# hidasib/GRU4Rec

Hardware: NVIDIA H100
Metric: mini-batches/sec (higher is better)
Workload: dtype f32

## Files before the change

### gru4rec_b200/csrc/g4r_fast.cuh

```cuda
#pragma once

constexpr int FK_THREADS = 512;
constexpr int FK_NW = FK_THREADS / 32;
constexpr int FK_G = 48;
constexpr int FK_CT = 32;
constexpr int FK_Q = FK_CT / FK_NW;
constexpr int FK_B = 32;
static_assert(FK_THREADS / 16 == FK_B, "statistics mapping: 16 threads per lane");
constexpr int FK_LDS = 132;


__device__ __forceinline__ void red_release_add(unsigned int* p, unsigned int v) {
  asm volatile("red.release.gpu.global.add.u32 [%0], %1;" :: "l"(p), "r"(v) : "memory");
}
__device__ __forceinline__ unsigned int atom_acqrel_add(unsigned int* p, unsigned int v) {
  unsigned int old;
  asm volatile("atom.acq_rel.gpu.global.add.u32 %0, [%1], %2;" : "=r"(old) : "l"(p), "r"(v) : "memory");
  return old;
}
__device__ __forceinline__ void wait_ge(const unsigned int* p, unsigned int target) {
  while (ld_acquire_u32(p) < target) { }
}
__device__ __forceinline__ uint32_t smem_u32(const void* p) { return (uint32_t)__cvta_generic_to_shared(p); }
__device__ __forceinline__ void mbar_init(uint64_t* bar, unsigned int count) {
// ... 604 lines not shown
  }
}
template <class SM>
__device__ __forceinline__ void fk_dsy(SM& sm, int M, int nj, int kw) {
  for (int t = threadIdx.x; t < nj * kw; t += FK_THREADS) {
    const int jj = t / kw, q4 = t % kw;
    float4 d = make_float4(0.f, 0.f, 0.f, 0.f);
    for (int bb = 0; bb < M; bb++) {
      const float4 y = ld4(sm.sY + bb * FK_LDS + q4 * 4);
      const float g = sm.sG[jj * FK_B + bb];
      d.x = fmaf(g, y.x, d.x); d.y = fmaf(g, y.y, d.y); d.z = fmaf(g, y.z, d.z); d.w = fmaf(g, y.w, d.w);
    }
    st4(sm.sD + jj * FK_LDS + q4 * 4, d);
  }
}
template <class SM>
__device__ __forceinline__ void fk_update_rows(const ModelDev& md, SM& sm, int buf, int nj, int kw) {
  const int lane = threadIdx.x & 31, warp = threadIdx.x >> 5, ldL = md.ldL;
  const bool ada = md.adapt == G4R_ADAPT_ADAGRAD, mom = md.mom > 0.f;
  for (int j = warp; j < nj; j += FK_NW) {
    const int item = sm.sIt[buf][j];
    if (j > 0 && sm.sIt[buf][j - 1] == item) continue;
    int je = j + 1;
    while (je < nj && sm.sIt[buf][je] == item) je++;
    if (lane < kw) {
      const float4 p0 = ld4(sm.sS + j * FK_LDS + lane * 4), z = make_float4(0.f, 0.f, 0.f, 0.f);
      RowChain<float4> u;
      u.begin(p0, p0, ada ? ld4(sm.sAcc + j * FK_LDS + lane * 4) : z, mom ? ld4(sm.sVel + j * FK_LDS + lane * 4) : z);
      for (int k = j; k < je; k++) u.add(md, ld4(sm.sD + k * FK_LDS + lane * 4), ada, mom);
      const size_t off = (size_t)item * ldL + lane * 4;
      st4(md.Wy + off, u.ps);
      if (ada) st4(md.Wy_acc + off, u.al);
      if (mom) st4(md.Wy_vel + off, u.vl);
    }
    if (lane == 0) {
      RowChain<float> u;
      u.begin(sm.sByP[j], sm.sByP[j], sm.sByA[j], sm.sByV[j]);
      for (int k = j; k < je; k++) u.add(md, sm.sDby[k], ada, mom);
      md.By[item] = u.ps;
      if (ada) md.By_acc[item] = u.al;
      if (mom) md.By_vel[item] = u.vl;
    }
  }
}
template <class SM>
__device__ __forceinline__ void fk_dby(SM& sm, int M, int nj) {
  const int lane = threadIdx.x & 31, warp = threadIdx.x >> 5;
  for (int jj = warp; jj < nj; jj += FK_NW) {
    float a = (lane < M) ? sm.sG[jj * FK_B + lane] : 0.f;
    a = warp_sum(a);
    if (lane == 0) sm.sDby[jj] = a;
  }
}
struct FkPartner { int nj, it; float g[2]; };
__device__ __forceinline__ FkPartner fk_partner_fetch(const ModelDev& md, int s, int g, int M) {
  const int tid = threadIdx.x;
  const int* cbeg = md.pCbeg + (size_t)s * (md.NCH + 1);
  const int cb = g < md.NCH ? cbeg[g] : 0;
  FkPartner r;
  r.nj = g < md.NCH ? cbeg[g + 1] - cb : 0;
  r.it = (tid < r.nj) ? md.pItem[(size_t)s * md.NP + cb + tid] : 0;
#pragma unroll
  for (int u = 0; u < 2; u++) {
    const int i = u * FK_THREADS + tid, jj = i / FK_B, b = i % FK_B;
    r.g[u] = (jj < r.nj && b < M) ? md.O[(size_t)(cb + jj) * md.Bld + b] : 0.f;
  }
  return r;
}
template <class SM>
__device__ int fk_partner_stage(const ModelDev& md, SM& sm, const FkPartner& r, int buf, int M, int kw) {
  static_assert(FK_CT * FK_B == 2 * FK_THREADS, "fk_partner_fetch: two dL/do entries per thread");
  const int tid = threadIdx.x, lane = tid & 31, warp = tid >> 5, nj = r.nj;
  const bool ada = md.adapt == G4R_ADAPT_ADAGRAD, mom = md.mom > 0.f;
  __syncthreads();
  if (tid < FK_CT) sm.sIt[buf][tid] = r.it;
  sm.sG[tid] = r.g[0]; sm.sG[FK_THREADS + tid] = r.g[1];
  __syncthreads();
  for (int j = warp; j < nj; j += FK_NW) {
    const int it = sm.sIt[buf][j];
    const size_t off = (size_t)it * md.ldL + lane * 4;
    if (lane < kw) {
      st4(sm.sS + j * FK_LDS + lane * 4, ld4(md.Wy + off));
      if (ada) st4(sm.sAcc + j * FK_LDS + lane * 4, ld4(md.Wy_acc + off));
      if (mom) st4(sm.sVel + j * FK_LDS + lane * 4, ld4(md.Wy_vel + off));
    }
    if (lane == 0) { sm.sByP[j] = md.By[it]; sm.sByA[j] = ada ? md.By_acc[it] : 0.f; sm.sByV[j] = mom ? md.By_vel[it] : 0.f; }
  }
  asm volatile("fence.proxy.async.shared::cta;" ::: "memory");
  fk_dby(sm, M, nj);
  return nj;
}

#include "g4r_fastc.cuh"

template <bool CL>
__global__ void __launch_bounds__(FK_THREADS, 1) k_fast_t(int slot, int n_steps, FastSync* fs, unsigned long long* tstamp) {
  using SM = typename std::conditional<CL, FastSmemC, FastSmemR>::type;
  extern __shared__ __align__(128) unsigned char fk_raw[];
  SM& sm = *reinterpret_cast<SM*>(fk_raw);
  const ModelDev& md = MD;
  const LayerDev& ly = md.layer[0];
  const int cta = blockIdx.x, ncta = gridDim.x;
  const int tid = threadIdx.x, lane = tid & 31, warp = tid >> 5;
  const int chunk = cta;
  const bool has_chunk = chunk < md.NCH;
  const int G = CL ? (int)cl_size() : md.ldL / 4;
  const bool gru = cta < G;
  const bool pw = loss_pairwise(md.loss);
  const int ldL = md.ldL, B = md.B;
  const int kw = ldL / 4;
  uint64_t* bar = reinterpret_cast<uint64_t*>(&sm.mbar);
  unsigned int bar_epoch = 0, gepoch = 0, stats_target = 0;
  const int in_ctas = min(B, ncta - G);
  const int partner_of = (!CL && cta >= G + in_ctas && cta < 2 * G + in_ctas) ? cta - G - in_ctas : -1;
#ifdef G4R_CF_FINE
#define FK_FTS(s_) ((tstamp && cta == 0 && (s_) < 500 && n_steps >= 1000) ? tstamp + (size_t)((s_) + 500) * 16 : nullptr)
#define FK_STAMP_OK(s_) ((s_) < 500)
#else
#define FK_FTS(s_) ((unsigned long long*)nullptr)
#define FK_STAMP_OK(s_) true
#endif
#define FK_STAMP(k) do { if (tstamp && cta == 0 && tid == 0 && FK_STAMP_OK(s)) { unsigned long long t_; asm volatile("mov.u64 %0, %%globaltimer;" : "=l"(t_)); tstamp[(size_t)s * 16 + (k)] = t_; } } while (0)
  if (tid == 0) { mbar_init(bar, 1); asm volatile("fence.mbarrier_init.release.cluster;" ::: "memory"); }
  fk_load_idx(md, sm, 0, n_steps, chunk, 0);
  __syncthreads();
  fk_prefetch_rows(md, sm, 0, n_steps, 0, pw);
  ClusterCtx cc = {0, 1, 0, 0};
  if constexpr (CL) {
    if (gru) {
      cc = cf_init(md, sm);
      cf_load_resident(md, sm, cc);
      if (n_steps > 0) {
        fk_stage_lanes(md, sm, 0, md.wM[0]);
        cf_f1(md, sm, cc, 0, false, nullptr, 0u, nullptr);
        cf_f2(md, sm, cc, 0, nullptr);
        __syncthreads();
        if (tid == 0) red_release_add(&fs->h_ready, 1u);
      }
    }
  } else {
    if (gru) {
      fr_load_resident(md, sm, 4 * cta);
      if (n_steps > 0) {
        fk_stage_lanes(md, sm, 0, md.wM[0]);
        stage_rows4(sm.gH[0], FK_LDS, FK_B, kw, [&](int rr) -> const float* { const int sl = sm.gIdx[rr]; return sl >= 0 ? ly.H + (size_t)sl * ldL : nullptr; });
        fr_f1(md, sm, 0, 4 * cta, sm.gH[0], nullptr, 0u);
        fk_group_barrier(fs, gepoch, G);
        fr_f2(md, sm, 0, 4 * cta, sm.gH[0]);
        __syncthreads();
        if (tid == 0) red_release_add(&fs->h_ready, 1u);
      }
    }
  }
  for (int s = 0; s < n_steps; s++) {
    const int buf = s & 1;
    const int M = md.wM[s];
    const int sti = md.wSti[s];
    const int N = M + (sti >= 0 ? md.S : 0);
    FK_STAMP(0);
    fk_load_idx(md, sm, s + 1, n_steps, chunk, buf ^ 1);
    const bool gru_next = !CL && gru && s + 1 < n_steps;
    if (gru_next && tid < FK_B) {
      const int M1 = md.wM[s + 1];
      sm.gIdx[tid] = tid < M1 ? md.wSlot[(size_t)(s + 1) * B + tid] : -1;
      sm.gIdx[FK_B + tid] = tid < M1 ? md.wX[(size_t)(s + 1) * B + tid] : 0;
      sm.gIdx[2 * FK_B + tid] = tid < M1 ? md.wF[(size_t)(s + 1) * B + tid] : 0;
    }
    if (tid == 0) wait_ge(&fs->h_ready, (unsigned int)(s + 1) * (unsigned int)G);
    __syncthreads();
    stage_rows4(sm.sY, FK_LDS, FK_B, kw, [&](int rr) -> const float* { return rr < M ? ly.y + (size_t)rr * ldL : nullptr; });
    mbar_wait(bar, (unsigned int)(s & 1));
    __syncthreads();
    FK_STAMP(1);
    const int cb = sm.sCb[buf][0], ce = sm.sCb[buf][1];
    const int nj = ce - cb;
    if (pw) {
      for (int b = warp; b < FK_B; b += FK_NW) {
        if (b < M) {
          float a = 0.f;
          if (lane < kw) {
            const float4 y = ld4(sm.sY + b * FK_LDS + lane * 4), w = ld4(sm.sTW + b * FK_LDS + lane * 4);
            a = fmaf(w.x, y.x, a); a = fmaf(w.y, y.y, a); a = fmaf(w.z, y.z, a); a = fmaf(w.w, y.w, a);
          }
          a = warp_sum(a);
          if (lane == 0) sm.sT[b] = act_fwd(md.fact, a + sm.sTB[b]);
        }
      }
    }
    {
      float accq[FK_Q];
#pragma unroll
      for (int q = 0; q < FK_Q; q++) accq[q] = 0.f;
      const float* yr = sm.sY + lane * FK_LDS;
      for (int c4 = 0; c4 < kw; c4++) {
        const float4 y = ld4(yr + c4 * 4);
#pragma unroll
        for (int q = 0; q < FK_Q; q++) {
          if (warp + FK_NW * q < nj) {
            const float4 w = ld4(sm.sS + (warp + FK_NW * q) * FK_LDS + c4 * 4);
            accq[q] = fmaf(y.x, w.x, accq[q]); accq[q] = fmaf(y.y, w.y, accq[q]); accq[q] = fmaf(y.z, w.z, accq[q]); accq[q] = fmaf(y.w, w.w, accq[q]);
          }
        }
      }
      FK_STAMP(9);
#pragma unroll
      for (int q = 0; q < FK_Q; q++) {
        const int jj = warp + q * FK_NW;
        if (jj < nj && lane < M) sm.sO[jj * FK_B + lane] = accq[q] + sm.sBias[jj];
      }
      __syncthreads();
      {
        const int b = tid >> 4, sub = tid & 15;
        const bool okb = b < M;
        const int tc = okb ? sm.sTc[buf][b] : -1;
        const float t = (pw && okb) ? sm.sT[b] : 0.f;
        float yv[2]; bool use[2], ist[2];
        float mloc = -INFINITY;
        const bool smx = loss_softmaxneg(md.loss), xe = (md.loss == G4R_LOSS_XE || md.loss == G4R_LOSS_XE_LOGIT);
#pragma unroll
        for (int q = 0; q < 2; q++) {
          const int jj = sub + 16 * q;
          use[q] = okb && jj < nj;
          ist[q] = use[q] && (tc == cb + jj);
          const float o = use[q] ? sm.sO[jj * FK_B + b] : 0.f;
          yv[q] = xe ? o : act_fwd(md.fact, o);
          if (use[q] && (xe || (smx && !ist[q]))) mloc = fmaxf(mloc, yv[q]);
        }
#pragma unroll
        for (int o = 1; o < 16; o <<= 1) mloc = fmaxf(mloc, __shfl_xor_sync(0xffffffffu, mloc, o));
        float Z = 0.f, A = 0.f, Q = 0.f, D = 0.f, T = 0.f, has = 0.f;
#pragma unroll
        for (int q = 0; q < 2; q++) {
          if (!use[q]) continue;
          const float y = yv[q];
          if (ist[q]) has = 1.f;
          if (xe) { Z += expf(y - mloc); if (ist[q]) T = y; }
          else if (md.loss == G4R_LOSS_BPR_MAX) { if (!ist[q]) { const float e = expf(y - mloc), sg = sigmoidf_(t - y); Z += e; A += sg * e; Q += y * y * e; D += sg * (1.f - sg) * e; } }
          else if (md.loss == G4R_LOSS_TOP1_MAX) { if (!ist[q]) { const float e = expf(y - mloc), a1 = sigmoidf_(y - t), b1 = sigmoidf_(y * y); Z += e; A += (a1 + b1) * e; D += a1 * (1.f - a1) * e; } }
          else if (md.loss == G4R_LOSS_BPR) { const float sg = sigmoidf_(t - y); A += -logf(sg); if (!ist[q]) D += 1.f - sg; }
          else { const float a1 = sigmoidf_(y - t), b1 = sigmoidf_(y * y); A += a1 + b1; if (!ist[q]) D += a1 * (1.f - a1); }
        }
#pragma unroll
        for (int o = 1; o < 16; o <<= 1) {
          Z += __shfl_xor_sync(0xffffffffu, Z, o); A += __shfl_xor_sync(0xffffffffu, A, o); Q += __shfl_xor_sync(0xffffffffu, Q, o);
          D += __shfl_xor_sync(0xffffffffu, D, o); T += __shfl_xor_sync(0xffffffffu, T, o); has += __shfl_xor_sync(0xffffffffu, has, o);
        }
        if (has_chunk && okb && sub == 0) {
          float* st = md.stat + ((size_t)chunk * md.B + b) * G4R_NSTAT;
          st4(st, make_float4(mloc, Z, A, Q));
          st4(st + 4, make_float4(D, T, has > 0.f ? 1.f : 0.f, pw ? t : 0.f));
        }
      }
    }
    __syncthreads();
    FK_STAMP(10);
    bar_epoch += 1;
    if (tid == 0) { red_release_add(&fs->bar, 1u); wait_ge(&fs->bar, bar_epoch * (unsigned int)ncta); }
    __syncthreads();
    if (cta < M) {
      const int b = cta;
      const bool maxed = !(md.loss == G4R_LOSS_BPR || md.loss == G4R_LOSS_TOP1);
      float mc = -INFINITY, Z = 0.f, A = 0.f, Q = 0.f, D = 0.f, T = 0.f, has = 0.f, tt = 0.f;
      if (tid < md.NCH) {
        const float* st = md.stat + ((size_t)tid * md.B + b) * G4R_NSTAT;
        const float4 u = ld4(st), v = ld4(st + 4);
        mc = u.x; Z = u.y; A = u.z; Q = u.w; D = v.x; T = v.y; has = v.z;
        if (tid == 0) tt = v.w;
      }
      float mg = mc;
#pragma unroll
      for (int o = 1; o < 32; o <<= 1) mg = fmaxf(mg, __shfl_xor_sync(0xffffffffu, mg, o));
      if (lane == 0) sm.sPart[warp] = mg;
      __syncthreads();
      mg = sm.sPart[0];
      for (int w = 1; w < FK_NW; w++) mg = fmaxf(mg, sm.sPart[w]);
      if (loss_softmaxneg(md.loss)) mg = fmaxf(mg, 0.f);
      if (maxed) {
        const float sc = (mc == -INFINITY) ? 0.f : expf(mc - mg);
        Z *= sc; A *= sc; Q *= sc; D *= sc;
      }
#pragma unroll
      for (int o = 1; o < 32; o <<= 1) {
        Z += __shfl_xor_sync(0xffffffffu, Z, o); A += __shfl_xor_sync(0xffffffffu, A, o); Q += __shfl_xor_sync(0xffffffffu, Q, o);
        D += __shfl_xor_sync(0xffffffffu, D, o); T += __shfl_xor_sync(0xffffffffu, T, o); has += __shfl_xor_sync(0xffffffffu, has, o);
      }
      __syncthreads();
      if (lane == 0) { float* w = sm.sPart + 32 + warp * 8; w[0] = Z; w[1] = A; w[2] = Q; w[3] = D; w[4] = T; w[5] = has; w[6] = tt; }
      __syncthreads();
      if (tid == 0) {
        tt = sm.sPart[32 + 6];
        for (int w = 1; w < FK_NW; w++) { const float* q = sm.sPart + 32 + w * 8; Z += q[0]; A += q[1]; Q += q[2]; D += q[3]; T += q[4]; }
        const float m = mg;
        float* rs = md.RS + (size_t)b * G4R_NSTAT;
        float loss = 0.f, r0 = m, r1 = Z, r2 = 0.f, r3 = 0.f, r4 = 0.f, r5 = tt;
        if (md.loss == G4R_LOSS_XE) { const float pt = __fdiv_rn(expf(T - m), Z); loss = -logf(pt + G4R_EPS_LOG); r2 = pt; r5 = T; }
        else if (md.loss == G4R_LOSS_XE_LOGIT) { loss = logf(Z) - (T - m); r5 = T; }
        else if (md.loss == G4R_LOSS_BPR_MAX) { r2 = __fdiv_rn(A, Z); r3 = __fdiv_rn(Q, Z); r4 = __fdiv_rn(D, Z); loss = -logf(r2 + G4R_EPS_LOG) + md.bpreg * r3; }
        else if (md.loss == G4R_LOSS_TOP1_MAX) { r2 = __fdiv_rn(A, Z); r4 = __fdiv_rn(D, Z); loss = r2; }
        else if (md.loss == G4R_LOSS_BPR) { loss = A; r4 = D; }
        else { const float c = sigmoidf_(tt * tt); loss = (float)M * (__fdiv_rn(A, (float)N) - __fdiv_rn(c, (float)(M + md.S_cfg))); r4 = D; }
        st4(rs, make_float4(r0, r1, r2, r3));
        st4(rs + 4, make_float4(r4, r5, loss, 0.f));
        red_release_add(&fs->stats, 1u);
      }
    }
    stats_target += (unsigned int)M;
    if (tid == 0) wait_ge(&fs->stats, stats_target);
    __syncthreads();
    FK_STAMP(2);
    if (tid < M * 2) st4(sm.sRS + tid * 4, ld4(md.RS + tid * 4));
    __syncthreads();
    if (chunk == 0 && tid == 0) {
      float c = 0.f;
      for (int b = 0; b < M; b++) c += sm.sRS[b * 8 + 6];
      c = __fdiv_rn(c, (float)md.B);
      md.cost[s] = c;
      if (c != c) atomicExch(md.nanflag, 1);
    }
    FK_STAMP(11);
    for (int i = tid; i < FK_CT * FK_B; i += FK_THREADS) {
      const int jj = i / FK_B, b = i % FK_B;
      sm.sG[i] = (jj < nj && b < M) ? loss_grad_elem(md, sm.sRS + (size_t)b * 8, sm.sO[i], sm.sTc[buf][b] == cb + jj, M, N) : 0.f;
    }
    __syncthreads();
    if (!CL && gru) {
      for (int i = tid; i < nj * FK_B; i += FK_THREADS) {
        const int jj = i / FK_B, b = i % FK_B;
        if (b < M) md.O[(size_t)(cb + jj) * md.Bld + b] = sm.sG[i];
      }
    } else {
      fk_dby(sm, M, nj);
    }
    FK_STAMP(12);
    float* part = md.part + (size_t)(has_chunk ? chunk : 0) * md.B * ldL;
    if constexpr (CL) {
      if (has_chunk) { fk_dsy(sm, M, nj, kw); fk_part(sm, part, M, nj, ldL); }
      __syncthreads();
      FK_STAMP(13);
      fk_update_rows(md, sm, buf, nj, kw);
      if (has_chunk && nj == 0) for (int i = tid; i < M * ldL; i += FK_THREADS) part[i] = 0.f;
      __syncthreads();
      FK_STAMP(14);
      bar_epoch += 1;
      if (tid == 0) { red_release_add(&fs->bar, 1u); wait_ge(&fs->bar, bar_epoch * (unsigned int)ncta); }
      __syncthreads();
      FK_STAMP(3);
      fk_b1<CL>(md, sm, s, cta, ncta);
      __syncthreads();
      if (tid == 0) red_release_add(&fs->b1_done, 1u);
      FK_STAMP(15);
      fk_prefetch_rows(md, sm, s + 1, n_steps, buf ^ 1, pw);
      FK_STAMP(4);
      if (gru) {
        if (s + 1 < n_steps) fk_stage_lanes(md, sm, s + 1, md.wM[s + 1]);
        cf_backward(md, sm, cc, fs, s, ncta, s + 1 < n_steps, (tstamp && cta == 0 && FK_STAMP_OK(s)) ? tstamp + (size_t)s * 16 : nullptr, FK_FTS(s));
        FK_STAMP(6);
        if (s + 1 < n_steps) {
          cf_f1(md, sm, cc, s + 1, true, &fs->in_done, (unsigned int)(s + 1) * (unsigned int)in_ctas, FK_FTS(s));
          FK_STAMP(7);
          cf_f2(md, sm, cc, s + 1, FK_FTS(s));
          __syncthreads();
          if (tid == 0) red_release_add(&fs->h_ready, 1u);
        } else {
          cl_wait();
        }
        FK_STAMP(8);
      }
      if (!gru && cta < G + in_ctas) {
        const unsigned int tgt = (unsigned int)(s + 1) * (unsigned int)G;
        if (in_ctas == B && ly.ld3 / 4 <= FK_THREADS) fk_sparse_in_one(md, sm, s, cta - G, &fs->grp, tgt);
        else {
          if (tid == 0) wait_ge(&fs->grp, tgt);
          __syncthreads();
          for (int b = cta - G; b < B; b += in_ctas) { fk_sparse_in(md, sm, s, b); __syncthreads(); }
        }
        __syncthreads();
        if (tid == 0) red_release_add(&fs->in_done, 1u);
      }
    } else {
      if (has_chunk) fk_part(sm, part, M, nj, ldL);
      if (has_chunk && nj == 0) for (int i = tid; i < M * ldL; i += FK_THREADS) part[i] = 0.f;
      __syncthreads();
      FK_STAMP(13);
      bar_epoch += 1;
      if (tid == 0) { red_release_add(&fs->bar, 1u); wait_ge(&fs->bar, bar_epoch * (unsigned int)ncta); }
      __syncthreads();
      FK_STAMP(3);
      fk_b1<CL>(md, sm, s, cta, ncta);
      __syncthreads();
      if (tid == 0) red_release_add(&fs->b1_done, 1u);
      FK_STAMP(15);
      const bool nxt = s + 1 < n_steps;
      const unsigned int rows_target = (unsigned int)(s + 1) * (unsigned int)ncta;
      if (gru) {
        const int k0 = 4 * cta;
        const float* sHo = sm.gH[s & 1];
        float* hnext = sm.gH[(s + 1) & 1];
        if (nxt) stage_rows4(hnext, FK_LDS, FK_B, kw, [&](int rr) -> const float* { const int sl = sm.gIdx[rr]; return sl >= 0 ? ly.H + (size_t)sl * ldL : nullptr; });
        __syncthreads();
        FK_STAMP(14);
        if (tid == 0) { red_release_add(&fs->rows_done, 1u); wait_ge(&fs->b1_done, (unsigned int)(s + 1) * (unsigned int)ncta); }
        __syncthreads();
        FK_STAMP(4);
        fr_b2(md, sm, s, k0, sHo);
        __syncthreads();
        if (tid == 0) red_release_add(&fs->dvec_done, 1u);
        FK_STAMP(5);
        fr_dense(md, sm, s, k0, sHo);
        FK_STAMP(6);
        if (nxt) {
          fr_f1(md, sm, s + 1, k0, hnext, &fs->in_done, (unsigned int)(s + 1) * (unsigned int)in_ctas);
          fk_group_barrier(fs, gepoch, G);
          FK_STAMP(7);
          fr_f2(md, sm, s + 1, k0, hnext);
          __syncthreads();
          if (tid == 0) red_release_add(&fs->h_ready, 1u);
          if (tid == 0) wait_ge(&fs->rows_done, rows_target);
          __syncthreads();
          fk_prefetch_rows(md, sm, s + 1, n_steps, buf ^ 1, pw);
        }
        FK_STAMP(8);
      } else {
        const FkPartner pc = partner_of >= 0 ? fk_partner_fetch(md, s, partner_of, M) : FkPartner{0, 0, {0.f, 0.f}};
        for (int pass = 0, njp = nj; pass < (partner_of >= 0 ? 2 : 1); pass++) {
          if (pass == 1) njp = fk_partner_stage(md, sm, pc, buf, M, kw);
          fk_dsy(sm, M, njp, kw);
          __syncthreads();
          fk_update_rows(md, sm, buf, njp, kw);
        }
        __syncthreads();
        if (tid == 0) red_release_add(&fs->rows_done, 1u);
        if (cta < G + in_ctas) {
          const unsigned int tgt = (unsigned int)(s + 1) * (unsigned int)G;
          if (in_ctas == B && ly.ld3 / 4 <= FK_THREADS) fk_sparse_in_one(md, sm, s, cta - G, &fs->dvec_done, tgt);
          else {
            if (tid == 0) wait_ge(&fs->dvec_done, tgt);
            __syncthreads();
            for (int b = cta - G; b < B; b += in_ctas) { fk_sparse_in(md, sm, s, b); __syncthreads(); }
          }
          __syncthreads();
          if (tid == 0) red_release_add(&fs->in_done, 1u);
        }
        if (nxt) {
          if (tid == 0) wait_ge(&fs->rows_done, rows_target);
          __syncthreads();
          fk_prefetch_rows(md, sm, s + 1, n_steps, buf ^ 1, pw);
        }
      }
    }
  }
  if constexpr (CL) { if (gru) cf_store_resident(md, sm, cc); }
  else { if (gru) fr_store_resident(md, sm, 4 * cta); }
#undef FK_STAMP
}
```

### gru4rec_b200/csrc/g4r_lib.cu

```cuda
#include <cuda_runtime.h>
#include <algorithm>
#include <cmath>
#include <cstdio>
#include <cstring>
#include <map>
#include <mutex>
#include <string>
#include <vector>
#include "g4r_kernels.cuh"
#include "g4r_misc.cuh"

#define G4R_VERSION 100

static thread_local std::string g_create_error;
struct g4r_handle;
static void eval_release(g4r_handle* h);
static void sessions_release(g4r_handle* h);
static void mg_release(g4r_handle* h);
static void shard_release(g4r_handle* h);
static bool shard_eligible(const g4r_config& c, int n_sm);
static int shard_create(g4r_handle* h);
static bool tc_eligible(const g4r_config& c);
struct TensorInfo;
static int shard_set_tensor(g4r_handle* h, const TensorInfo& t, const float* host);
// ... 300 lines not shown
__global__ void __launch_bounds__(256) k_gather_in(int slot, const int* base, int off, int train) { phase_gather_in(MD, STEP_IDX, train != 0, blockIdx.x, gridDim.x); }
__global__ void __launch_bounds__(GEMM_THREADS) k_f1(int slot, const int* base, int off, int li, float* Hsrc) {
  __shared__ float sA[GK * (GB + 1)], sB[GK * (GB + 1)];
  phase_f1(MD, li, STEP_IDX, Hsrc, blockIdx.x, sA, sB);
}
__global__ void __launch_bounds__(GEMM_THREADS) k_f2(int slot, const int* base, int off, int li, float* Hsrc, int train) {
  __shared__ float sA[GK * (GB + 1)], sB[GK * (GB + 1)];
  phase_f2(MD, li, STEP_IDX, Hsrc, train != 0, blockIdx.x, sA, sB);
}
__global__ void __launch_bounds__(SC_THREADS) k_score(int slot, const int* base, int off) {
  extern __shared__ __align__(16) float smem[];
  phase_score(MD, STEP_IDX, blockIdx.x, smem);
}
__global__ void __launch_bounds__(256) k_stats(int slot, const int* base, int off) {
  extern __shared__ __align__(16) float smem[];
  phase_stats(MD, STEP_IDX, blockIdx.x, gridDim.x, smem);
}
__global__ void __launch_bounds__(SC_THREADS) k_lossgrad(int slot, const int* base, int off) {
  extern __shared__ __align__(16) float smem[];
  phase_lossgrad(MD, STEP_IDX, blockIdx.x, smem);
}
__global__ void __launch_bounds__(256) k_b1(int slot, const int* base, int off, int li, int nch) { phase_b1(MD, li, STEP_IDX, blockIdx.x, gridDim.x, nch); }
__global__ void __launch_bounds__(GEMM_THREADS) k_b2(int slot, const int* base, int off, int li) {
  __shared__ float sA[GK * (GB + 1)], sB[GK * (GB + 1)];
  phase_b2(MD, li, STEP_IDX, blockIdx.x, sA, sB);
}
__global__ void __launch_bounds__(GEMM_THREADS) k_b3(int slot, const int* base, int off, int li) {
  __shared__ float sA[GK * (GB + 1)], sB[GK * (GB + 1)];
  phase_b3(MD, li, STEP_IDX, blockIdx.x, sA, sB);
}
__global__ void __launch_bounds__(GEMM_THREADS) k_dense(int slot, const int* base, int off, int li) {
  __shared__ float sA[GK * (GB + 1)], sB[GK * (GB + 1)];
  phase_dense(MD, li, STEP_IDX, blockIdx.x, sA, sB);
}
__global__ void __launch_bounds__(128) k_sparse_in(int slot, const int* base, int off, int apply_pass) { phase_sparse_in(MD, STEP_IDX, blockIdx.x, apply_pass != 0); }
__global__ void __launch_bounds__(256) k_stats2a(int slot, const int* base, int off) { phase_stats2a(MD, STEP_IDX, blockIdx.x); }
__global__ void __launch_bounds__(256) k_stats2b(int slot, const int* base, int off) {
  __shared__ float smem[64];
  phase_stats2b(MD, STEP_IDX, blockIdx.x, gridDim.x, smem);
}
__global__ void __launch_bounds__(1024) k_gradnorm(int slot, const int* base, int off, const float* dense_flat, size_t dense_count, float* gscale) {
  __shared__ float smem[32];
  phase_gradnorm(MD, STEP_IDX, dense_flat, dense_count, gscale, smem);
}
__global__ void __launch_bounds__(SC_THREADS) k_apply_rows(int slot, const int* base, int off) { phase_apply_rows(MD, STEP_IDX, blockIdx.x); }
__global__ void __launch_bounds__(256) k_apply_dense(int slot, float* p, float* acc, float* vel, const float* g, int n) {
  const int i = blockIdx.x * blockDim.x + threadIdx.x;
  if (i < n) dense_update(MD, p + i, acc ? acc + i : nullptr, vel ? vel + i : nullptr, g[i], (size_t)n);
}
__global__ void k_advance(int* base, int n) { if (threadIdx.x == 0 && blockIdx.x == 0) *base += n; }

#include "g4r_persistent.cuh"
#include "g4r_fast.cuh"

constexpr int FC_CLUSTER = 8;
static cudaError_t fastc_config(cudaLaunchConfig_t& lc, cudaLaunchAttribute* attrs, int n_attr_coop, int grid, cudaStream_t st) {
  lc = cudaLaunchConfig_t{};
  lc.gridDim = dim3(grid); lc.blockDim = dim3(FK_THREADS); lc.dynamicSmemBytes = sizeof(FastSmemC); lc.stream = st;
  attrs[0].id = cudaLaunchAttributeClusterDimension;
  attrs[0].val.clusterDim.x = FC_CLUSTER; attrs[0].val.clusterDim.y = 1; attrs[0].val.clusterDim.z = 1;
  attrs[1].id = cudaLaunchAttributeCooperative; attrs[1].val.cooperative = 1;
  lc.attrs = attrs; lc.numAttrs = 1 + n_attr_coop;
  return cudaSuccess;
}
static int fastc_max_grid(int n_sm) {
  if (cudaFuncSetAttribute(k_fast_t<true>, cudaFuncAttributeMaxDynamicSharedMemorySize, (int)sizeof(FastSmemC)) != cudaSuccess) { cudaGetLastError(); return 0; }
  cudaLaunchConfig_t lc; cudaLaunchAttribute attrs[2];
  fastc_config(lc, attrs, 0, (n_sm / FC_CLUSTER) * FC_CLUSTER, nullptr);
  int ncl = 0;
  if (cudaOccupancyMaxActiveClusters(&ncl, k_fast_t<true>, &lc) != cudaSuccess) { cudaGetLastError(); return 0; }
  return std::min(ncl, n_sm / FC_CLUSTER) * FC_CLUSTER;
}
static cudaError_t fastc_launch(int grid, cudaStream_t st, void** args) {
  static int coop_ok = 1;
  cudaLaunchConfig_t lc; cudaLaunchAttribute attrs[2];
  if (coop_ok) {
    fastc_config(lc, attrs, 1, grid, st);
    cudaError_t e = cudaLaunchKernelExC(&lc, (const void*)k_fast_t<true>, args);
    if (e == cudaSuccess) return e;
    cudaGetLastError();
    coop_ok = 0;
  }
  fastc_config(lc, attrs, 0, grid, st);
  return cudaLaunchKernelExC(&lc, (const void*)k_fast_t<true>, args);
}

static std::mutex g_smem_mutex;
static std::map<const void*, int> g_smem_limit;
static cudaError_t raise_smem_limit(const void* func, size_t bytes) {
  std::lock_guard<std::mutex> lk(g_smem_mutex);
  int& cur = g_smem_limit[func];
  if ((int)bytes <= cur) return cudaSuccess;
  const cudaError_t e = cudaFuncSetAttribute(func, cudaFuncAttributeMaxDynamicSharedMemorySize, (int)bytes);
  if (e == cudaSuccess) cur = (int)bytes;
  return e;
}

static int tiles2(int cols, int rows) { return ((cols + GB - 1) / GB) * ((rows + GB - 1) / GB); }

#include "g4r_eval_tc.cuh"
#include "g4r_tcstep.cuh"
static bool tc_eligible(const g4r_config& c) {
  if (!c.constrained_embedding || c.n_layers != 1 || c.batch_size > 256 || (c.layers[0] & 3)) return false;
  if (c.adapt > G4R_ADAPT_ADAGRAD || c.grad_cap > 0.f || c.smoothing != 0.f || c.world_size > 1) return false;
  return c.step_mode == 4 || (c.step_mode >= 1 && c.step_mode <= 3 && c.layers[0] >= 160);
}
// ... 200 lines not shown
  if (h->stream) cudaStreamSynchronize(h->stream);
  sessions_release(h);
  eval_release(h);
  if (h->ts_buf) { delete static_cast<TsBuf*>(h->ts_buf); h->ts_buf = nullptr; }
  shard_release(h);
  mg_release(h);
  if (h->graphU) cudaGraphExecDestroy(h->graphU);
  if (h->graph1) cudaGraphExecDestroy(h->graph1);
  slot_free(h->slot);
  if (h->ev0) cudaEventDestroy(h->ev0);
  if (h->ev1) cudaEventDestroy(h->ev1);
  if (h->hX) cudaFreeHost(h->hX);
  if (h->hY) cudaFreeHost(h->hY);
  if (h->hSlot) cudaFreeHost(h->hSlot);
  if (h->hM) cudaFreeHost(h->hM);
  if (h->hSti) cudaFreeHost(h->hSti);
  if (h->hF) cudaFreeHost(h->hF);
  if (h->hG) cudaFreeHost(h->hG);
  if (h->hCost) cudaFreeHost(h->hCost);
  if (h->hFlags) cudaFreeHost(h->hFlags);
  if (h->own_ws && h->ws) cudaFree(h->ws);
  if (h->ts_dbg) { ts_print_stamps(h); cudaFree(h->ts_dbg); }
  if (h->side) cudaStreamDestroy(h->side);
  if (h->side2) cudaStreamDestroy(h->side2);
  for (cudaEvent_t e : h->ts_ev) if (e) cudaEventDestroy(e);
  if (h->stream) cudaStreamDestroy(h->stream);
  delete h;
  return G4R_OK;
}

extern "C" int g4r_create(const g4r_config* cfg, void* device_workspace, size_t workspace_bytes, g4r_handle** out) {
  if (!cfg || !out) { g_create_error = "null argument"; return G4R_ERR_INVALID; }
  std::string err;
  int rc = validate_config(*cfg, err);
  if (rc) { g_create_error = err; return rc; }
  int dev_count = 0;
  cudaError_t ce = cudaGetDeviceCount(&dev_count);
  if (ce != cudaSuccess || dev_count <= cfg->device) {
    g_create_error = "no CUDA device available: libg4r has no CPU path";
    return G4R_ERR_CUDA;
  }
  g4r_handle* h = new g4r_handle();
  h->cfg = *cfg;
  auto bail = [&](int code, const std::string& m) { g_create_error = m; g4r_destroy(h); return code; };
  if (cudaSetDevice(cfg->device) != cudaSuccess) return bail(G4R_ERR_CUDA, "cudaSetDevice failed");
  cudaDeviceProp prop;
  if (cudaGetDeviceProperties(&prop, cfg->device) != cudaSuccess) return bail(G4R_ERR_CUDA, "cudaGetDeviceProperties failed");
  h->n_sm = prop.multiProcessorCount;
  int chunk_cap = h->n_sm;
  if (cfg->step_mode == 3) {
    h->fastc_grid = fastc_max_grid(h->n_sm);
    if (h->fastc_grid >= FC_CLUSTER * 2) chunk_cap = std::min(chunk_cap, h->fastc_grid);
  }
  size_t need = 0;
  { Carver cv{nullptr, 0, true}; layout(*cfg, cv, nullptr, chunk_cap); need = align_up(cv.off, 256) + 256; }
  if (device_workspace) {
    if (workspace_bytes < need) return bail(G4R_ERR_INVALID, "workspace too small");
    h->ws = (char*)device_workspace; h->own_ws = false;
  } else {
    if (cudaMalloc(&h->ws, need) != cudaSuccess) return bail(G4R_ERR_CUDA, "cudaMalloc of workspace failed");
    h->own_ws = true;
  }
  h->ws_bytes = need;
  if (cudaStreamCreateWithFlags(&h->stream, cudaStreamNonBlocking) != cudaSuccess) return bail(G4R_ERR_CUDA, "stream create failed");
  cudaEventCreate(&h->ev0); cudaEventCreate(&h->ev1);
  if (cudaStreamCreateWithFlags(&h->side, cudaStreamNonBlocking) != cudaSuccess || cudaStreamCreateWithFlags(&h->side2, cudaStreamNonBlocking) != cudaSuccess) return bail(G4R_ERR_CUDA, "stream create failed");
  for (cudaEvent_t& e : h->ts_ev) cudaEventCreateWithFlags(&e, cudaEventDisableTiming);
  if (cudaMemsetAsync(h->ws, 0, need, h->stream) != cudaSuccess) return bail(G4R_ERR_CUDA, "memset failed");
  char* base = (char*)align_up((size_t)h->ws, 256);
  Carver cv{base, 0, false};
  layout(*cfg, cv, h, chunk_cap);
  h->slot = slot_alloc();
  if (h->slot < 0) return bail(G4R_ERR_STATE, "too many live g4r handles in this process");
  if (h->two_pass) h->md.export_only = 1;
  if (slot_upload(h->slot, h->md, h->stream) != cudaSuccess) return bail(G4R_ERR_CUDA, "constant upload failed");
  const int B = cfg->batch_size, CAP = h->CAP;
  bool ok = true;
  ok &= cudaMallocHost(&h->hX, (size_t)CAP * B * sizeof(int)) == cudaSuccess;
  ok &= cudaMallocHost(&h->hY, (size_t)CAP * B * sizeof(int)) == cudaSuccess;
  ok &= cudaMallocHost(&h->hSlot, (size_t)CAP * B * sizeof(int)) == cudaSuccess;
  ok &= cudaMallocHost(&h->hF, (size_t)CAP * B) == cudaSuccess;
  ok &= cudaMallocHost(&h->hM, (size_t)CAP * sizeof(int)) == cudaSuccess;
  ok &= cudaMallocHost(&h->hSti, (size_t)CAP * sizeof(int)) == cudaSuccess;
  ok &= cudaMallocHost(&h->hG, (size_t)CAP * sizeof(uint32_t)) == cudaSuccess;
  ok &= cudaMallocHost(&h->hCost, (size_t)CAP * sizeof(float)) == cudaSuccess;
  if (!ok) return bail(G4R_ERR_CUDA, "pinned host allocation failed");
  h->pk_smem = std::max(std::max(score_smem_bytes(h->md.Bld), lossgrad_smem_bytes(h->md.Bld, h->md.ldL)), (size_t)2 * GK * (GB + 1) * sizeof(float));
  if (raise_smem_limit((const void*)k_score, score_smem_bytes(h->md.Bld)) != cudaSuccess ||
      raise_smem_limit((const void*)k_lossgrad, lossgrad_smem_bytes(h->md.Bld, h->md.ldL)) != cudaSuccess ||
      raise_smem_limit((const void*)k_plan, (size_t)h->npow2 * 8 + 1024) != cudaSuccess ||
      raise_smem_limit((const void*)k_persistent, h->pk_smem) != cudaSuccess)
    return bail(G4R_ERR_INVALID, "this shape needs more shared memory per block than the device offers (batch_size / layer width / n_sample too large for the step scratch)");
  {
    int per_sm = 0;
    cudaOccupancyMaxActiveBlocksPerMultiprocessor(&per_sm, k_persistent, PK_THREADS, h->pk_smem);
    int coop = 0; cudaDeviceGetAttribute(&coop, cudaDevAttrCooperativeLaunch, cfg->device);
    h->pk_blocks = (per_sm >= 1 && coop) ? h->n_sm : 0;
  }
  {
    const ModelDev& m = h->md;
    raise_smem_limit((const void*)k_fast_t<false>, sizeof(FastSmemR));
    int per_sm = 0;
    cudaOccupancyMaxActiveBlocksPerMultiprocessor(&per_sm, k_fast_t<false>, FK_THREADS, sizeof(FastSmemR));
    const bool plain_opt = m.adapt <= G4R_ADAPT_ADAGRAD && !h->phase_only;
    h->fast_ok = plain_opt && h->pk_blocks > 0 && per_sm >= 1 && m.mode == 0 && m.n_layers == 1 && m.ldL <= 128 && m.B <= FK_B && h->n_sm >= FK_G + 1 && m.NCH <= 160 &&
                 2 * m.L <= FK_W1 * FK_G && m.L <= FK_W2 * FK_G &&
                 h->pk_blocks >= 2 * (m.ldL / 4) + std::min(m.B, h->pk_blocks - m.ldL / 4) &&
                 (m.adapt == G4R_ADAPT_ADAGRAD ? m.Wy_acc != nullptr : true);
    h->fastc_ok = plain_opt && cfg->step_mode == 3 && h->fastc_grid >= FC_CLUSTER * 2 && m.mode == 0 && m.n_layers == 1 && m.ldL <= 128 && m.B <= FK_B &&
                  m.NCH <= h->fastc_grid && (m.adapt == G4R_ADAPT_ADAGRAD ? m.Wy_acc != nullptr : true);
    cudaMallocHost(&h->hFlags, 4 * sizeof(int));
  }
  if (h->tc_ok) {
    if (ts_opt_in(h) != G4R_OK) return bail(G4R_ERR_CUDA, "k_ts_gemm: shared memory / cluster opt-in failed");
    h->fast_ok = false; h->fastc_ok = false;
  }
  if (cfg->step_mode == 1 && h->pk_blocks == 0) return bail(G4R_ERR_INVALID, "persistent mode unavailable (cooperative launch / shared memory)");
  if (h->md.shardR > 0) {
    const int src = shard_create(h);
    if (src) return bail(src, h->err);
    h->fast_ok = false; h->fastc_ok = false;
  }
  if (cudaStreamSynchronize(h->stream) != cudaSuccess) return bail(G4R_ERR_CUDA, "init sync failed");
  *out = h;
  return G4R_OK;
}

extern "C" void* g4r_stream(g4r_handle* h) { return h ? (void*)h->stream : nullptr; }
extern "C" int64_t g4r_kernel_launches(const g4r_handle* h) { return h ? h->launches : 0; }

static TensorInfo* find_tensor(g4r_handle* h, const char* name) {
  auto it = h->tensors.find(name ? name : "");
  return it == h->tensors.end() ? nullptr : &it->second;
}
extern "C" int g4r_tensor_shape(g4r_handle* h, const char* name, int64_t* rows, int64_t* cols) {
  if (!h) return G4R_ERR_INVALID;
  TensorInfo* t = find_tensor(h, name);
  if (!t) FAIL(G4R_ERR_INVALID, std::string("unknown tensor ") + (name ? name : "(null)"));
  if (rows) *rows = t->rows;
  if (cols) *cols = t->cols;
  return G4R_OK;
}
extern "C" int g4r_set_tensor(g4r_handle* h, const char* name, const float* host, int64_t rows, int64_t cols) {
  if (!h || !host) return G4R_ERR_INVALID;
  TensorInfo* t = find_tensor(h, name);
  if (!t) FAIL(G4R_ERR_INVALID, std::string("unknown tensor ") + (name ? name : "(null)"));
  if (rows != t->rows || cols != t->cols) FAIL(G4R_ERR_INVALID, std::string("shape mismatch for ") + name);
  cudaSetDevice(h->cfg.device);
  if (t->ptr == h->md.Wy || t->ptr == h->md.By) h->wy_version++;
  if (t->sharded) return shard_set_tensor(h, *t, host);
  CK(cudaMemcpy2DAsync(t->ptr, t->ld * sizeof(float), host, cols * sizeof(float), cols * sizeof(float), rows, cudaMemcpyHostToDevice, h->stream));
  CK(cudaStreamSynchronize(h->stream));
  return G4R_OK;
}
extern "C" int g4r_get_tensor(g4r_handle* h, const char* name, float* host, int64_t rows, int64_t cols) {
  if (!h || !host) return G4R_ERR_INVALID;
  TensorInfo* t = find_tensor(h, name);
  if (!t) FAIL(G4R_ERR_INVALID, std::string("unknown tensor ") + (name ? name : "(null)"));
  if (rows != t->rows || cols != t->cols) FAIL(G4R_ERR_INVALID, std::string("shape mismatch for ") + name);
  cudaSetDevice(h->cfg.device);
// ... 548 lines not shown
```

Baseline: 30470.

## Dedicate GRU CTAs to recurrence and give output chunks only to column CTAs

In the non-cluster fast kernel, the first G CTAs now run only the GRU backward/forward recurrence. Only the remaining CTAs own output-column chunks, and the chunk count is capped at n_sm minus G to match. This removes the earlier scheme where GRU CTAs also scored chunks, wrote dL/do to global memory, and had partner CTAs re-stage and update those rows. The cost is fewer CTAs doing scoring and row updates, so each column CTA does more, while the GRU CTAs no longer sit on the scoring critical path. The fast-path eligibility check is reworked into a shared shape predicate to match.

```diff
diff --git a/gru4rec_b200/csrc/g4r_fast.cuh b/gru4rec_b200/csrc/g4r_fast.cuh
--- a/gru4rec_b200/csrc/g4r_fast.cuh
+++ b/gru4rec_b200/csrc/g4r_fast.cuh
@@ -680,45 +680,6 @@
     if (lane == 0) sm.sDby[jj] = a;
   }
 }
-struct FkPartner { int nj, it; float g[2]; };
-__device__ __forceinline__ FkPartner fk_partner_fetch(const ModelDev& md, int s, int g, int M) {
-  const int tid = threadIdx.x;
-  const int* cbeg = md.pCbeg + (size_t)s * (md.NCH + 1);
-  const int cb = g < md.NCH ? cbeg[g] : 0;
-  FkPartner r;
-  r.nj = g < md.NCH ? cbeg[g + 1] - cb : 0;
-  r.it = (tid < r.nj) ? md.pItem[(size_t)s * md.NP + cb + tid] : 0;
-#pragma unroll
-  for (int u = 0; u < 2; u++) {
-    const int i = u * FK_THREADS + tid, jj = i / FK_B, b = i % FK_B;
-    r.g[u] = (jj < r.nj && b < M) ? md.O[(size_t)(cb + jj) * md.Bld + b] : 0.f;
-  }
-  return r;
-}
-template <class SM>
-__device__ int fk_partner_stage(const ModelDev& md, SM& sm, const FkPartner& r, int buf, int M, int kw) {
-  static_assert(FK_CT * FK_B == 2 * FK_THREADS, "fk_partner_fetch: two dL/do entries per thread");
-  const int tid = threadIdx.x, lane = tid & 31, warp = tid >> 5, nj = r.nj;
-  const bool ada = md.adapt == G4R_ADAPT_ADAGRAD, mom = md.mom > 0.f;
-  __syncthreads();
-  if (tid < FK_CT) sm.sIt[buf][tid] = r.it;
-  sm.sG[tid] = r.g[0]; sm.sG[FK_THREADS + tid] = r.g[1];
-  __syncthreads();
-  for (int j = warp; j < nj; j += FK_NW) {
-    const int it = sm.sIt[buf][j];
-    const size_t off = (size_t)it * md.ldL + lane * 4;
-    if (lane < kw) {
-      st4(sm.sS + j * FK_LDS + lane * 4, ld4(md.Wy + off));
-      if (ada) st4(sm.sAcc + j * FK_LDS + lane * 4, ld4(md.Wy_acc + off));
-      if (mom) st4(sm.sVel + j * FK_LDS + lane * 4, ld4(md.Wy_vel + off));
-    }
-    if (lane == 0) { sm.sByP[j] = md.By[it]; sm.sByA[j] = ada ? md.By_acc[it] : 0.f; sm.sByV[j] = mom ? md.By_vel[it] : 0.f; }
-  }
-  asm volatile("fence.proxy.async.shared::cta;" ::: "memory");
-  fk_dby(sm, M, nj);
-  return nj;
-}
-
 #include "g4r_fastc.cuh"
 
 template <bool CL>
@@ -730,17 +691,18 @@
   const LayerDev& ly = md.layer[0];
   const int cta = blockIdx.x, ncta = gridDim.x;
   const int tid = threadIdx.x, lane = tid & 31, warp = tid >> 5;
-  const int chunk = cta;
-  const bool has_chunk = chunk < md.NCH;
   const int G = CL ? (int)cl_size() : md.ldL / 4;
   const bool gru = cta < G;
+  const bool col = CL || !gru;
+  const int chunk = CL ? cta : cta - G;
+  const int ncol = CL ? ncta : ncta - G;
+  const bool has_chunk = col && chunk < md.NCH;
   const bool pw = loss_pairwise(md.loss);
   const int ldL = md.ldL, B = md.B;
   const int kw = ldL / 4;
   uint64_t* bar = reinterpret_cast<uint64_t*>(&sm.mbar);
   unsigned int bar_epoch = 0, gepoch = 0, stats_target = 0;
   const int in_ctas = min(B, ncta - G);
-  const int partner_of = (!CL && cta >= G + in_ctas && cta < 2 * G + in_ctas) ? cta - G - in_ctas : -1;
 #ifdef G4R_CF_FINE
 #define FK_FTS(s_) ((tstamp && cta == 0 && (s_) < 500 && n_steps >= 1000) ? tstamp + (size_t)((s_) + 500) * 16 : nullptr)
 #define FK_STAMP_OK(s_) ((s_) < 500)
@@ -748,11 +710,11 @@
 #define FK_FTS(s_) ((unsigned long long*)nullptr)
 #define FK_STAMP_OK(s_) true
 #endif
-#define FK_STAMP(k) do { if (tstamp && cta == 0 && tid == 0 && FK_STAMP_OK(s)) { unsigned long long t_; asm volatile("mov.u64 %0, %%globaltimer;" : "=l"(t_)); tstamp[(size_t)s * 16 + (k)] = t_; } } while (0)
+#define FK_STAMP(k) do { if (tstamp && cta == ((CL || ((k) >= 4 && (k) <= 8)) ? 0 : G) && tid == 0 && FK_STAMP_OK(s)) { unsigned long long t_; asm volatile("mov.u64 %0, %%globaltimer;" : "=l"(t_)); tstamp[(size_t)s * 16 + (k)] = t_; } } while (0)
   if (tid == 0) { mbar_init(bar, 1); asm volatile("fence.mbarrier_init.release.cluster;" ::: "memory"); }
-  fk_load_idx(md, sm, 0, n_steps, chunk, 0);
-  __syncthreads();
-  fk_prefetch_rows(md, sm, 0, n_steps, 0, pw);
+  if (col) fk_load_idx(md, sm, 0, n_steps, chunk, 0);
+  __syncthreads();
+  if (col) fk_prefetch_rows(md, sm, 0, n_steps, 0, pw);
   ClusterCtx cc = {0, 1, 0, 0};
   if constexpr (CL) {
     if (gru) {
@@ -786,7 +748,7 @@
     const int sti = md.wSti[s];
     const int N = M + (sti >= 0 ? md.S : 0);
     FK_STAMP(0);
-    fk_load_idx(md, sm, s + 1, n_steps, chunk, buf ^ 1);
+    if (col) fk_load_idx(md, sm, s + 1, n_steps, chunk, buf ^ 1);
     const bool gru_next = !CL && gru && s + 1 < n_steps;
     if (gru_next && tid < FK_B) {
       const int M1 = md.wM[s + 1];
@@ -796,6 +758,35 @@
     }
     if (tid == 0) wait_ge(&fs->h_ready, (unsigned int)(s + 1) * (unsigned int)G);
     __syncthreads();
+    if constexpr (!CL) {
+      if (!col) {
+        const bool nxt = s + 1 < n_steps;
+        const int k0 = 4 * cta;
+        const float* sHo = sm.gH[s & 1];
+        float* hnext = sm.gH[(s + 1) & 1];
+        if (nxt) stage_rows4(hnext, FK_LDS, FK_B, kw, [&](int rr) -> const float* { const int sl = sm.gIdx[rr]; return sl >= 0 ? ly.H + (size_t)sl * ldL : nullptr; });
+        __syncthreads();
+        if (tid == 0) wait_ge(&fs->b1_done, (unsigned int)(s + 1) * (unsigned int)ncol);
+        __syncthreads();
+        FK_STAMP(4);
+        fr_b2(md, sm, s, k0, sHo);
+        __syncthreads();
+        if (tid == 0) red_release_add(&fs->dvec_done, 1u);
+        FK_STAMP(5);
+        fr_dense(md, sm, s, k0, sHo);
+        FK_STAMP(6);
+        if (nxt) {
+          fr_f1(md, sm, s + 1, k0, hnext, &fs->in_done, (unsigned int)(s + 1) * (unsigned int)in_ctas);
+          fk_group_barrier(fs, gepoch, G);
+          FK_STAMP(7);
+          fr_f2(md, sm, s + 1, k0, hnext);
+          __syncthreads();
+          if (tid == 0) red_release_add(&fs->h_ready, 1u);
+        }
+        FK_STAMP(8);
+        continue;
+      }
+    }
     stage_rows4(sm.sY, FK_LDS, FK_B, kw, [&](int rr) -> const float* { return rr < M ? ly.y + (size_t)rr * ldL : nullptr; });
     mbar_wait(bar, (unsigned int)(s & 1));
     __syncthreads();
@@ -883,10 +874,10 @@
     __syncthreads();
     FK_STAMP(10);
     bar_epoch += 1;
-    if (tid == 0) { red_release_add(&fs->bar, 1u); wait_ge(&fs->bar, bar_epoch * (unsigned int)ncta); }
+    if (tid == 0) { red_release_add(&fs->bar, 1u); wait_ge(&fs->bar, bar_epoch * (unsigned int)ncol); }
     __syncthreads();
-    if (cta < M) {
-      const int b = cta;
+    if (chunk < M) {
+      const int b = chunk;
       const bool maxed = !(md.loss == G4R_LOSS_BPR || md.loss == G4R_LOSS_TOP1);
       float mc = -INFINITY, Z = 0.f, A = 0.f, Q = 0.f, D = 0.f, T = 0.f, has = 0.f, tt = 0.f;
       if (tid < md.NCH) {
@@ -951,14 +942,7 @@
       sm.sG[i] = (jj < nj && b < M) ? loss_grad_elem(md, sm.sRS + (size_t)b * 8, sm.sO[i], sm.sTc[buf][b] == cb + jj, M, N) : 0.f;
     }
     __syncthreads();
-    if (!CL && gru) {
-      for (int i = tid; i < nj * FK_B; i += FK_THREADS) {
-        const int jj = i / FK_B, b = i % FK_B;
-        if (b < M) md.O[(size_t)(cb + jj) * md.Bld + b] = sm.sG[i];
-      }
-    } else {
-      fk_dby(sm, M, nj);
-    }
+    fk_dby(sm, M, nj);
     FK_STAMP(12);
     float* part = md.part + (size_t)(has_chunk ? chunk : 0) * md.B * ldL;
     if constexpr (CL) {
@@ -1011,69 +995,34 @@
       __syncthreads();
       FK_STAMP(13);
       bar_epoch += 1;
-      if (tid == 0) { red_release_add(&fs->bar, 1u); wait_ge(&fs->bar, bar_epoch * (unsigned int)ncta); }
+      if (tid == 0) { red_release_add(&fs->bar, 1u); wait_ge(&fs->bar, bar_epoch * (unsigned int)ncol); }
       __syncthreads();
       FK_STAMP(3);
-      fk_b1<CL>(md, sm, s, cta, ncta);
+      fk_b1<CL>(md, sm, s, chunk, ncol);
       __syncthreads();
       if (tid == 0) red_release_add(&fs->b1_done, 1u);
       FK_STAMP(15);
-      const bool nxt = s + 1 < n_steps;
-      const unsigned int rows_target = (unsigned int)(s + 1) * (unsigned int)ncta;
-      if (gru) {
-        const int k0 = 4 * cta;
-        const float* sHo = sm.gH[s & 1];
-        float* hnext = sm.gH[(s + 1) & 1];
-        if (nxt) stage_rows4(hnext, FK_LDS, FK_B, kw, [&](int rr) -> const float* { const int sl = sm.gIdx[rr]; return sl >= 0 ? ly.H + (size_t)sl * ldL : nullptr; });
-        __syncthreads();
-        FK_STAMP(14);
-        if (tid == 0) { red_release_add(&fs->rows_done, 1u); wait_ge(&fs->b1_done, (unsigned int)(s + 1) * (unsigned int)ncta); }
-        __syncthreads();
-        FK_STAMP(4);
-        fr_b2(md, sm, s, k0, sHo);
-        __syncthreads();
-        if (tid == 0) red_release_add(&fs->dvec_done, 1u);
-        FK_STAMP(5);
-        fr_dense(md, sm, s, k0, sHo);
-        FK_STAMP(6);
-        if (nxt) {
-          fr_f1(md, sm, s + 1, k0, hnext, &fs->in_done, (unsigned int)(s + 1) * (unsigned int)in_ctas);
-          fk_group_barrier(fs, gepoch, G);
-          FK_STAMP(7);
-          fr_f2(md, sm, s + 1, k0, hnext);
+      fk_dsy(sm, M, nj, kw);
+      __syncthreads();
+      if (chunk < in_ctas) {
+        const unsigned int tgt = (unsigned int)(s + 1) * (unsigned int)G;
+        if (in_ctas == B && ly.ld3 / 4 <= FK_THREADS) fk_sparse_in_one(md, sm, s, chunk, &fs->dvec_done, tgt);
+        else {
+          if (tid == 0) wait_ge(&fs->dvec_done, tgt);
           __syncthreads();
-          if (tid == 0) red_release_add(&fs->h_ready, 1u);
-          if (tid == 0) wait_ge(&fs->rows_done, rows_target);
-          __syncthreads();
-          fk_prefetch_rows(md, sm, s + 1, n_steps, buf ^ 1, pw);
-        }
-        FK_STAMP(8);
-      } else {
-        const FkPartner pc = partner_of >= 0 ? fk_partner_fetch(md, s, partner_of, M) : FkPartner{0, 0, {0.f, 0.f}};
-        for (int pass = 0, njp = nj; pass < (partner_of >= 0 ? 2 : 1); pass++) {
-          if (pass == 1) njp = fk_partner_stage(md, sm, pc, buf, M, kw);
-          fk_dsy(sm, M, njp, kw);
-          __syncthreads();
-          fk_update_rows(md, sm, buf, njp, kw);
+          for (int b = chunk; b < B; b += in_ctas) { fk_sparse_in(md, sm, s, b); __syncthreads(); }
         }
         __syncthreads();
-        if (tid == 0) red_release_add(&fs->rows_done, 1u);
-        if (cta < G + in_ctas) {
-          const unsigned int tgt = (unsigned int)(s + 1) * (unsigned int)G;
-          if (in_ctas == B && ly.ld3 / 4 <= FK_THREADS) fk_sparse_in_one(md, sm, s, cta - G, &fs->dvec_done, tgt);
-          else {
-            if (tid == 0) wait_ge(&fs->dvec_done, tgt);
-            __syncthreads();
-            for (int b = cta - G; b < B; b += in_ctas) { fk_sparse_in(md, sm, s, b); __syncthreads(); }
-          }
-          __syncthreads();
-          if (tid == 0) red_release_add(&fs->in_done, 1u);
-        }
-        if (nxt) {
-          if (tid == 0) wait_ge(&fs->rows_done, rows_target);
-          __syncthreads();
-          fk_prefetch_rows(md, sm, s + 1, n_steps, buf ^ 1, pw);
-        }
+        if (tid == 0) red_release_add(&fs->in_done, 1u);
+      }
+      fk_update_rows(md, sm, buf, nj, kw);
+      __syncthreads();
+      FK_STAMP(14);
+      if (tid == 0) red_release_add(&fs->rows_done, 1u);
+      if (s + 1 < n_steps) {
+        if (tid == 0) wait_ge(&fs->rows_done, (unsigned int)(s + 1) * (unsigned int)ncol);
+        __syncthreads();
+        fk_prefetch_rows(md, sm, s + 1, n_steps, buf ^ 1, pw);
       }
     }
   }
diff --git a/gru4rec_b200/csrc/g4r_lib.cu b/gru4rec_b200/csrc/g4r_lib.cu
--- a/gru4rec_b200/csrc/g4r_lib.cu
+++ b/gru4rec_b200/csrc/g4r_lib.cu
@@ -376,6 +376,14 @@
 
 #include "g4r_persistent.cuh"
 #include "g4r_fast.cuh"
+
+static bool fast_shape(const g4r_config& c, int n_sm) {
+  const int L = c.layers[0], ldL = round4(L);
+  const bool smoothing = (c.loss == G4R_LOSS_XE || c.loss == G4R_LOSS_XE_LOGIT) && c.smoothing > 0.f;
+  return c.step_mode == 2 && c.adapt <= G4R_ADAPT_ADAGRAD && !(c.grad_cap > 0.f) && !smoothing && model_mode(c) == 0 && c.n_layers == 1 &&
+         ldL <= 128 && c.batch_size <= FK_B && 2 * L <= FK_W1 * FK_G && L <= FK_W2 * FK_G && n_sm >= FK_G + 1 &&
+         n_sm - ldL / 4 >= c.batch_size && !tc_eligible(c) && !shard_eligible(c, n_sm);
+}
 
 constexpr int FC_CLUSTER = 8;
 static cudaError_t fastc_config(cudaLaunchConfig_t& lc, cudaLaunchAttribute* attrs, int n_attr_coop, int grid, cudaStream_t st) {
@@ -682,6 +690,7 @@
     h->fastc_grid = fastc_max_grid(h->n_sm);
     if (h->fastc_grid >= FC_CLUSTER * 2) chunk_cap = std::min(chunk_cap, h->fastc_grid);
   }
+  if (fast_shape(*cfg, h->n_sm)) chunk_cap = h->n_sm - round4(cfg->layers[0]) / 4;
   size_t need = 0;
   { Carver cv{nullptr, 0, true}; layout(*cfg, cv, nullptr, chunk_cap); need = align_up(cv.off, 256) + 256; }
   if (device_workspace) {
@@ -733,9 +742,7 @@
     int per_sm = 0;
     cudaOccupancyMaxActiveBlocksPerMultiprocessor(&per_sm, k_fast_t<false>, FK_THREADS, sizeof(FastSmemR));
     const bool plain_opt = m.adapt <= G4R_ADAPT_ADAGRAD && !h->phase_only;
-    h->fast_ok = plain_opt && h->pk_blocks > 0 && per_sm >= 1 && m.mode == 0 && m.n_layers == 1 && m.ldL <= 128 && m.B <= FK_B && h->n_sm >= FK_G + 1 && m.NCH <= 160 &&
-                 2 * m.L <= FK_W1 * FK_G && m.L <= FK_W2 * FK_G &&
-                 h->pk_blocks >= 2 * (m.ldL / 4) + std::min(m.B, h->pk_blocks - m.ldL / 4) &&
+    h->fast_ok = plain_opt && fast_shape(*cfg, h->n_sm) && h->pk_blocks == h->n_sm && per_sm >= 1 && m.NCH <= h->pk_blocks - m.ldL / 4 && m.NCH <= 160 &&
                  (m.adapt == G4R_ADAPT_ADAGRAD ? m.Wy_acc != nullptr : true);
     h->fastc_ok = plain_opt && cfg->step_mode == 3 && h->fastc_grid >= FC_CLUSTER * 2 && m.mode == 0 && m.n_layers == 1 && m.ldL <= 128 && m.B <= FK_B &&
                   m.NCH <= h->fastc_grid && (m.adapt == G4R_ADAPT_ADAGRAD ? m.Wy_acc != nullptr : true);
```

Result: faster. 32590, median of 6 (+6.9%).
